# tnestmeyer/reflectance-filtering

Hardware: AMD Instinct MI355X
Metric: megapixels/sec joint-bilateral sigma_c=20 sigma_s=22 @1080p (higher is better)
Workload: dtype f32

## Files before the change

### reflectance_filtering_amd/csrc/rf_jbf.hip

```cpp
#include <algorithm>
#include <atomic>
#include <mutex>
#include <vector>

#include "rf_jbf_common.hpp"
#include "rf_jbf_tables.hpp"
#include "rf_jbf_taploops.hpp"

namespace rf {
namespace {

constexpr int kTileW = 64;
constexpr int kMaxLds = 160 * 1024;
constexpr int kTlw2 = 144;
constexpr int kJbfMaxTiledR4 = 468;
constexpr int kJbfStageOnly = 0x1000, kJbfCompilerLoop = 0x2000, kJbfTile64Only = 0x4000;
constexpr int kJbfLookahead1 = 0x8000;
constexpr int kJbfNoMsad = 0x10000;
constexpr int kJbfVoteOnly = 0x20000;
constexpr int kJbfNoDeadSkip = 0x40000;

int jbf_debug_flags()
{
    return (debug_get(kDbgJbfStageOnly) ? kJbfStageOnly : 0) |
// ... 786 lines not shown
constexpr int kRaggedClasses = 4;
constexpr int kRaggedTh[kRaggedClasses] = {64, 32, 16, 128};
constexpr int kRaggedPitch144[kRaggedClasses] = {144, 208, 336, 136};

struct RaggedPlan {
    bool tiled = false;
    bool slab = false;
    Tile64Shape shape{};
    SlabShape slab_shape{};
    std::vector<JbfTileRec> recs[kRaggedClasses];
};

void plan_ragged(const JbfTables &t, int n, const int *heights, const int *widths, int src_cn,
                 int flags, int tune, RaggedPlan *plan)
{
    const int nz = t.lut_len < 256 * t.joint_cn ? t.lut_len - 1 : t.lut_len;
    if ((flags & RF_JBF_FORCE_GENERIC) || tune != 0)
        return;
    plan->tiled = tile64_choose(t, nz, src_cn, flags, &plan->shape);
    plan->slab = !plan->tiled && slab_choose(t, nz, src_cn, &plan->slab_shape);
    if (!plan->tiled && !plan->slab)
        return;
    const Tile64Shape &s = plan->shape;
    unsigned long long first = 0;
    for (int i = 0; i < n; i++) {
        const int h = heights[i], w = widths[i];
        Tile64Areas a{h, w, 0, 0, 0};
        if (plan->tiled && s.tlw == 144)
            a = tile64_areas(t, nz, s.grep, s.crep, src_cn, flags, h, w);
        const int area[kRaggedClasses][4] = {{0, a.rows_main, 0, a.cols_main},
                                             {a.rows_main, a.s32, 0, a.cols_main},
                                             {a.rows_main + a.s32, a.s16, 0, a.cols_main},
                                             {0, a.sx ? h : 0, a.cols_main, a.sx}};
        for (int c = 0; c < kRaggedClasses; c++) {
            const int th = kRaggedTh[c], tw = 4096 / th;
            for (int y = 0; y < area[c][1]; y += th)
                for (int x = 0; x < area[c][3]; x += tw)
                    plan->recs[c].push_back(
                        JbfTileRec{first, h, w, area[c][0] + y, area[c][2] + x, {0, 0}});
        }
        first += (unsigned long long)h * w;
    }
}

template <int SCN, int GREP, int CREP, int TLW, int TH>
int launch_tile64_ragged(const JbfTables &t, int nz, int crows, const uint8_t *joint,
                         const uint8_t *src, uint8_t *dst, const JbfTileRec *d_recs, size_t ntiles,
                         int jcn, int border, int flags, hipStream_t stream)
{
    if (ntiles == 0)
        return RF_OK;
    if (!launch_fits(ntiles, 1024))
        return fail(RF_E_UNSUPPORTED, "rf_jbf_ragged_u8: too many tiles for one launch");
    auto kern = jbf_tile64_kernel<SCN, GREP, CREP, TLW, TH, true>;
    RF_HIP_CHECK(hipFuncSetAttribute((const void *)kern, hipFuncAttributeMaxDynamicSharedMemorySize,
                                     kT64Lds));
    hipLaunchKernelGGL(kern, dim3((unsigned)ntiles), dim3(1024), kT64Lds, stream, joint, src, dst, 0,
                       0, jcn, t.radius, border, t.d_lut, nz, t.d_hw, t.d_swsym, t.sw_len, d_recs, 0,
                       flags, crows, 0, 0, JbfNoTileFlags{});
    return RF_OK;
}

template <int SCN, int GREP, int CREP, int TLW>
int launch_ragged(const JbfTables &t, int nz, const RaggedPlan &plan, const uint8_t *joint,
                  const uint8_t *src, uint8_t *dst, const JbfTileRec *const *d_recs, int jcn,
                  int border, int flags, hipStream_t stream)
{
    int rc = launch_tile64_ragged<SCN, GREP, CREP, TLW, 64>(t, nz, plan.shape.crows, joint, src, dst,
                                                            d_recs[0], plan.recs[0].size(), jcn,
                                                            border, flags, stream);
    if constexpr (TLW == 144) {
        if (rc == RF_OK)
            rc = launch_tile64_ragged<SCN, GREP, CREP, 208, 32>(t, nz, 32, joint, src, dst, d_recs[1],
                                                                plan.recs[1].size(), jcn, border,
                                                                flags, stream);
        if constexpr (SCN == 1) {
            if (rc == RF_OK)
                rc = launch_tile64_ragged<1, GREP, CREP, 336, 16>(t, nz, 32, joint, src, dst,
                                                                  d_recs[2], plan.recs[2].size(), jcn,
                                                                  border, flags, stream);
            if (rc == RF_OK)
                rc = launch_tile64_ragged<1, GREP, CREP, 136, 128>(t, nz, 32, joint, src, dst,
                                                                   d_recs[3], plan.recs[3].size(),
                                                                   jcn, border, flags, stream);
        }
    }
    return rc;
}

template <int GREP, int TLW, bool kRagged = false>
__global__ __launch_bounds__(1024) void jbf_slab_kernel(
    const uint8_t *__restrict__ joint, const uint8_t *__restrict__ src, uint8_t *__restrict__ dst,
    int h, int w, int jcn, int scn, int radius, int border, const float *__restrict__ lut, int nz,
    const int *__restrict__ hwtab, const float *__restrict__ swsym, int sw_len,
    typename JbfTilesArg<kRagged>::type tiles_x, int tiles_per_img, int flags, int crows_g, int slab_g,
    int crows_c, int slab_c)
{
    constexpr int NT = 1024, Q4 = TLW / 4, QW = 16;
    static_assert(TLW % 32 == 16, "row pitch keeps the rows of a half-wave on disjoint banks");
    extern __shared__ __align__(16) unsigned char smem[];
    int *flag_word = reinterpret_cast<int *>(smem);
    uint32_t *tile4 = reinterpret_cast<uint32_t *>(smem + 16);
    const int tid = threadIdx.x;
    if (tid == 0)
        *flag_word = 3;
    const int tile_id = xcd_contiguous_tile((int)blockIdx.x, (int)gridDim.x);
    int tile_y0, tile_x0;
    size_t img;
    if constexpr (kRagged) {
        const JbfTileRec *rec = tiles_x + tile_id;
        img = (size_t)rec->first;
        h = rec->h;
        w = rec->w;
        tile_y0 = rec->tile_y0;
        tile_x0 = rec->tile_x0;
    } else {
        const int img_idx = tile_id / tiles_per_img;
        const int t_in_img = tile_id - img_idx * tiles_per_img;
        tile_y0 = (t_in_img / tiles_x) * 64;
        tile_x0 = (t_in_img % tiles_x) * 64;
        img = (size_t)img_idx * h * w;
    }
    const int r4 = (radius + 3) & ~3;
    const int tx = tid % QW, ty = tid / QW;
    float *lut_g = reinterpret_cast<float *>(smem + kT64Lds - nz * GREP * 4);
    for (int i = tid; i < nz * GREP; i += NT)
        lut_g[i] = lut[i / GREP];
    const uint32_t lut_lane_addr = lds_addr(lut_g) + (uint32_t)(tid & (GREP - 1)) * 4u;
    const uint32_t tile_lane_addr = lds_addr(tile4) + (uint32_t)tx * 4u;
    int all_grey = scn == 1;
    if (scn == 3) {
        int grey = 1;
        const int rows_all = min(64, h - tile_y0) + 2 * radius;
        for (int item = tid; item < rows_all * Q4; item += NT) {
            const int ry = item / Q4, k = item - ry * Q4;
            const int gy = border_interpolate(tile_y0 - radius + ry, h, border);
            uint32_t jv[4], sv[4];
            load_tile_quad(joint, src, img, gy, tile_x0 - r4 + 4 * k, w, jcn, scn, border, jv, sv);
#pragma unroll
            for (int u = 0; u < 4; u++)
                grey &= (int)(((sv[u] ^ (sv[u] >> 8)) & 0xffffu) == 0u);
        }
        all_grey = __builtin_amdgcn_readfirstlane(block_all2(grey, 1, flag_word) & 1);
    }
    const bool rgb6 = !all_grey && crows_c > 0;
    const int crows = rgb6 ? crows_c : crows_g, slab_rows = rgb6 ? slab_c : slab_g;
    const bool active = tid < QW * crows;
    for (int y0 = tile_y0; y0 < tile_y0 + 64 && y0 < h; y0 += crows) {
        for (int c = 0; c < (all_grey || rgb6 ? 1 : scn); c++) {
            uint32_t jc[kPix];
            float sum1[kPix][1], sum3[kPix][3], wsum[kPix];
            {
                uint32_t jv[4], sv[4];
                load_tile_quad(joint, src, img, min(y0 + ty, h - 1), tile_x0 + 4 * tx, w, jcn, scn, border,
                               jv, sv);
#pragma unroll
                for (int p = 0; p < kPix; p++) {
                    jc[p] = jv[p] & 0x00ffffffu;
                    sum1[p][0] = sum3[p][0] = sum3[p][1] = sum3[p][2] = 0.f;
                    wsum[p] = 0.f;
                }
            }
            const bool msad = !(flags & kJbfNoMsad) && jbf_wave_takes_msad(jc, active);
            for (int i0 = -radius; i0 <= radius; i0 += slab_rows) {
                const int i1 = min(i0 + slab_rows - 1, radius);
                const int tlh = crows + (i1 - i0);
                uint16_t *plane_b = reinterpret_cast<uint16_t *>(tile4 + (size_t)tlh * TLW);
                __syncthreads();
                for (int item = tid; item < tlh * Q4; item += NT) {
                    const int ry = item / Q4, k = item - ry * Q4;
                    const int gy = border_interpolate(y0 + i0 + ry, h, border);
                    uint32_t jv[4], sv[4];
                    load_tile_quad(joint, src, img, gy, tile_x0 - r4 + 4 * k, w, jcn, scn, border, jv, sv);
#pragma unroll
                    for (int u = 0; u < 4; u++) {
                        tile4[ry * TLW + u * Q4 + k] = jv[u] | (((sv[u] >> (8 * c)) & 0xffu) << 24);
                        if (rgb6)
                            plane_b[ry * TLW + u * Q4 + k] = (uint16_t)(sv[u] >> 8);
                    }
                }
                __syncthreads();
                if (active) {
                    if (rgb6 && msad)
                        jbf_tap_loop_rgb6<GREP, TLW, true, true>(lut_lane_addr, swsym, tile_lane_addr,
                                                                 lds_addr(plane_b) + (uint32_t)tx * 2u, jc, ty,
                                                                 radius, r4, sw_len, hwtab, sum3, wsum, i0, i1,
                                                                 -i0);
                    else if (rgb6)
                        jbf_tap_loop_rgb6<GREP, TLW, true>(lut_lane_addr, swsym, tile_lane_addr,
                                                           lds_addr(plane_b) + (uint32_t)tx * 2u, jc, ty,
                                                           radius, r4, sw_len, hwtab, sum3, wsum, i0, i1, -i0);
                    else if (msad)
                        jbf_tap_loop_grey4_la2<GREP, TLW, false, true, true>(lut_lane_addr, swsym,
                                                                             tile_lane_addr, jc, ty, radius, r4,
                                                                             sw_len, hwtab, sum1, wsum, i0, i1,
                                                                             -i0);
                    else
                        jbf_tap_loop_grey4_la2<GREP, TLW, false, true>(lut_lane_addr, swsym, tile_lane_addr,
                                                                       jc, ty, radius, r4, sw_len, hwtab,
                                                                       sum1, wsum, i0, i1, -i0);
                }
            }
            if (active) {
                if (rgb6)
                    store_quad<3, 3>(dst, img, y0 + ty, tile_x0 + 4 * tx, h, w, sum3, wsum, flags);
                else if (scn == 1)
                    store_quad<1, 1>(dst, img, y0 + ty, tile_x0 + 4 * tx, h, w, sum1, wsum, flags);
                else if (all_grey)
                    store_quad<1, 3>(dst, img, y0 + ty, tile_x0 + 4 * tx, h, w, sum1, wsum, flags);
                else
                    store_quad_channel(dst, img, y0 + ty, tile_x0 + 4 * tx, h, w, c, sum1, wsum, flags);
            }
        }
    }
}

void slab_fits(const JbfTables &t, int nz, int grep, int tlw, int texel_bytes, int *crows, int *slab_rows)
{
    *crows = *slab_rows = 0;
    if (2 * t.r4 + 64 + 8 > tlw)
        return;
    const long long rows =
        ((long long)kT64Lds - 16 - (long long)nz * grep * 4) / ((long long)tlw * texel_bytes);
    for (int cr : {64, 32, 16}) {
        const long long sl = rows - cr + 1;
        if (sl >= (cr == 16 ? 8 : 24)) {
            *crows = cr;
            *slab_rows = (int)std::min<long long>(sl, 2 * t.radius + 1);
            return;
        }
    }
}

#define RF_SLAB_PITCHES(X)                                                                    \
    X(68, 208) X(84, 240) X(100, 272) X(116, 304) X(132, 336) X(164, 400) X(212, 496) X(276, 624) \
    X(372, 816) X(kJbfMaxTiledR4, 1008)

bool slab_choose(const JbfTables &t, int nz, int src_cn, SlabShape *out)
{
    if (t.r4 <= 52 || t.r4 > kJbfMaxTiledR4)
        return false;
    SlabShape s{};
#define RF_PITCH(R4_, TLW_) \
    if (!s.tlw && t.r4 <= R4_) \
        s.tlw = TLW_;
    RF_SLAB_PITCHES(RF_PITCH)
#undef RF_PITCH
    for (int g : {16, 8}) {
        int cr, sl;
        slab_fits(t, nz, g, s.tlw, 4, &cr, &sl);
        if (cr > s.crows_g)
            s.crows_g = cr, s.slab_g = sl, s.grep = g;
    }
    if (s.crows_g == 0)
        return false;
    if (src_cn == 3)
        slab_fits(t, nz, s.grep, s.tlw, 6, &s.crows_c, &s.slab_c);
    *out = s;
    return true;
}

template <int GREP, int TLW>
int launch_slab(const JbfTables &t, int nz, int crows, int slab_rows, int crows_c, int slab_c,
                const uint8_t *joint, const uint8_t *src, uint8_t *dst, int n, int h, int w, int jcn,
                int scn, int border, int flags, hipStream_t stream)
{
    const int tiles_x = ceil_div(w, 64), tiles_y = ceil_div(h, 64);
    const long long blocks = (long long)tiles_x * tiles_y * n;
    if (!launch_fits(blocks, 1024))
        return fail(RF_E_UNSUPPORTED, "rf_jbf_u8: batch too large for one launch");
    auto kern = jbf_slab_kernel<GREP, TLW>;
    RF_HIP_CHECK(hipFuncSetAttribute((const void *)kern, hipFuncAttributeMaxDynamicSharedMemorySize,
                                     kT64Lds));
    hipLaunchKernelGGL(kern, dim3((unsigned)blocks), dim3(1024), kT64Lds, stream, joint, src, dst, h,
                       w, jcn, scn, t.radius, border, t.d_lut, nz, t.d_hw, t.d_swsym, t.sw_len,
                       tiles_x, tiles_x * tiles_y, flags, crows, slab_rows, crows_c, slab_c);
    return RF_OK;
}

template <int GREP, int TLW>
int launch_slab_ragged(const JbfTables &t, int nz, const SlabShape &s, const uint8_t *joint,
                       const uint8_t *src, uint8_t *dst, const JbfTileRec *d_recs, size_t ntiles,
                       int jcn, int scn, int border, int flags, hipStream_t stream)
{
    if (ntiles == 0)
        return RF_OK;
    if (!launch_fits(ntiles, 1024))
        return fail(RF_E_UNSUPPORTED, "rf_jbf_ragged_u8: too many tiles for one launch");
    auto kern = jbf_slab_kernel<GREP, TLW, true>;
    RF_HIP_CHECK(hipFuncSetAttribute((const void *)kern, hipFuncAttributeMaxDynamicSharedMemorySize,
                                     kT64Lds));
    hipLaunchKernelGGL(kern, dim3((unsigned)ntiles), dim3(1024), kT64Lds, stream, joint, src, dst, 0,
                       0, jcn, scn, t.radius, border, t.d_lut, nz, t.d_hw, t.d_swsym, t.sw_len,
                       d_recs, 0, flags, s.crows_g, s.slab_g, s.crows_c, s.slab_c);
    return RF_OK;
}

int tile64x2_slab_rows(int nz, int grep, int tlw)
{
    const int rows = (kT64x2Lds - nz * grep * 4) / (tlw * 4);
    return rows >= 64 ? rows - 64 + 1 : 0;
}

template <int GREP, int TLW>
__global__ __launch_bounds__(1024, 8) void jbf_tile64x2_kernel(
    const uint8_t *__restrict__ joint, const uint8_t *__restrict__ src, uint8_t *__restrict__ dst,
    int h, int w, int jcn, int scn, int radius, int border, const float *__restrict__ lut, int nz,
    const int *__restrict__ hwtab, const float *__restrict__ swsym, int sw_len, int tiles_x,
    int tiles_per_img, int flags, int slab_rows, uint8_t *__restrict__ tile_flags)
{
    constexpr int NT = 1024, Q4 = TLW / 4, QW = 16;
    static_assert(TLW % 32 == 16, "row pitch keeps the rows of a half-wave on disjoint banks");
    extern __shared__ __align__(16) unsigned char smem[];
    int *flag_word = reinterpret_cast<int *>(smem);
    uint32_t *tile4 = reinterpret_cast<uint32_t *>(smem);
    const int tid = threadIdx.x;
    if (tid == 0)
        *flag_word = 3;
    __syncthreads();
    const int tile_id = xcd_contiguous_tile((int)blockIdx.x, (int)gridDim.x);
    const int img_idx = tile_id / tiles_per_img;
    const int t_in_img = tile_id - img_idx * tiles_per_img;
    const int tile_y0 = (t_in_img / tiles_x) * 64;
    const int tile_x0 = (t_in_img % tiles_x) * 64;
    const size_t img = (size_t)img_idx * h * w;
    const int r4 = (radius + 3) & ~3;
    const int tx = tid % QW, ty = tid / QW;
    int grey_joint = 1;
    if (flags & kJbfVoteOnly) {
        int grey = 1;
        const int rows_all = 64 + 2 * radius;
        for (int item = tid; item < rows_all * Q4; item += NT) {
            const int ry = item / Q4, k = item - ry * Q4;
            const int gy = border_interpolate(tile_y0 - radius + ry, h, border);
            uint32_t jv[4], sv[4];
            load_tile_quad(joint, src, img, gy, tile_x0 - r4 + 4 * k, w, jcn, scn, border, jv, sv);
#pragma unroll
            for (int u = 0; u < 4; u++) {
                if (scn == 3)
                    grey &= (int)(((sv[u] ^ (sv[u] >> 8)) & 0xffffu) == 0u);
                if (jcn == 3)
                    grey_joint &= (int)(((jv[u] ^ (jv[u] >> 8)) & 0xffffu) == 0u);
            }
        }
        const int bits = block_all2(grey, grey_joint, flag_word);
        if (tid == 0)
            tile_flags[tile_id] = (uint8_t)(((bits & 1) ? 0 : 1) | (bits & 2));
        return;
    }
    if (tile_flags) {
        const int byte = __builtin_amdgcn_readfirstlane((int)tile_flags[tile_id]);
        if (byte & 1)
            return;
        grey_joint = (byte >> 1) & 1;
    }
    float *lut_g = reinterpret_cast<float *>(smem + kT64x2Lds - nz * GREP * 4);
    for (int i = tid; i < nz * GREP; i += NT)
        lut_g[i] = lut[i / GREP];
    const uint32_t lut_lane_addr = lds_addr(lut_g) + (uint32_t)(tid & (GREP - 1)) * 4u;
    const uint32_t tile_lane_addr = lds_addr(tile4) + (uint32_t)tx * 4u;
    const bool j1 = grey_joint != 0;
    const uint32_t j1_scale = (uint32_t)(jcn == 1 ? 1 : 3) * (GREP * 4u);
    uint32_t jc[kPix];
    float sum1[kPix][1], wsum[kPix];
    {
        uint32_t jv[4], sv[4];
        load_tile_quad(joint, src, img, border_interpolate(tile_y0 + ty, h, border), tile_x0 + 4 * tx, w, jcn,
                       scn, border, jv, sv);
#pragma unroll
        for (int p = 0; p < kPix; p++) {
            jc[p] = j1 ? (jv[p] & 0xffu) * j1_scale : jv[p] & 0x00ffffffu;
            sum1[p][0] = 0.f;
            wsum[p] = 0.f;
        }
    }
    const bool msad = !j1 && !(flags & kJbfNoMsad) && jbf_wave_takes_msad(jc);
    const bool live_wave =
        __builtin_amdgcn_readfirstlane(tile_y0 + (ty & ~3)) < h || (flags & kJbfNoDeadSkip) != 0;
    for (int i0 = -radius; i0 <= radius; i0 += slab_rows) {
        const int i1 = min(i0 + slab_rows - 1, radius);
        const int tlh = 64 + (i1 - i0);
        __syncthreads();
        for (int item = tid; item < tlh * Q4; item += NT) {
            const int ry = item / Q4, k = item - ry * Q4;
            const int gy = border_interpolate(tile_y0 + i0 + ry, h, border);
            uint32_t jv[4], sv[4];
            load_tile_quad(joint, src, img, gy, tile_x0 - r4 + 4 * k, w, jcn, scn, border, jv, sv);
#pragma unroll
            for (int u = 0; u < 4; u++) {
                const uint32_t jfield = j1 ? (jv[u] & 0xffu) * j1_scale : jv[u];
                tile4[ry * TLW + u * Q4 + k] = jfield | (sv[u] << 24);
            }
        }
        __syncthreads();
        if (!live_wave)
            continue;
        if (j1)
            jbf_tap_loop_grey4_la2<GREP, TLW, true, true>(lut_lane_addr, swsym, tile_lane_addr, jc, ty,
                                                          radius, r4, sw_len, hwtab, sum1, wsum, i0, i1, -i0);
        else if (msad)
            jbf_tap_loop_grey4_la2<GREP, TLW, false, true, true>(lut_lane_addr, swsym, tile_lane_addr, jc,
                                                                 ty, radius, r4, sw_len, hwtab, sum1, wsum,
                                                                 i0, i1, -i0);
        else
            jbf_tap_loop_grey4_la2<GREP, TLW, false, true>(lut_lane_addr, swsym, tile_lane_addr, jc, ty,
                                                           radius, r4, sw_len, hwtab, sum1, wsum, i0, i1,
                                                           -i0);
    }
    if (scn == 1)
        store_quad<1, 1>(dst, img, tile_y0 + ty, tile_x0 + 4 * tx, h, w, sum1, wsum, flags);
    else
        store_quad<1, 3>(dst, img, tile_y0 + ty, tile_x0 + 4 * tx, h, w, sum1, wsum, flags);
}

struct TileFlagBuf {
    int dev;
    hipStream_t stream;
    uint8_t *p;
    size_t bytes;
};
std::mutex g_tf_mu;
std::vector<TileFlagBuf> g_tf;
std::vector<uint8_t *> g_tf_retired;
constexpr size_t kTileFlagStreams = 16;
std::atomic<int> g_two_wg_calls{0};

size_t tile_flag_bytes(size_t tiles)
{
    size_t b = 4096;
    while (b < tiles)
        b <<= 1;
    return b;
}

int get_tile_flags(int dev, hipStream_t stream, size_t tiles, uint8_t **out)
{
    *out = nullptr;
    std::lock_guard<std::mutex> lock(g_tf_mu);
    size_t at = g_tf.size();
    for (size_t i = 0; i < g_tf.size(); i++)
        if (g_tf[i].dev == dev && g_tf[i].stream == stream)
            at = i;
    if (at < g_tf.size() && g_tf[at].bytes >= tiles) {
        *out = g_tf[at].p;
        return RF_OK;
    }
    hipStreamCaptureStatus st = hipStreamCaptureStatusNone;
    if (hipStreamIsCapturing(stream, &st) != hipSuccess || st != hipStreamCaptureStatusNone) {
        (void)hipGetLastError();
        return RF_OK;
    }
    if (at == g_tf.size() && g_tf.size() >= kTileFlagStreams)
        return RF_OK;
    uint8_t *p = nullptr;
    {
        CaptureRelax relax;
        RF_HIP_CHECK(hipMalloc(&p, tile_flag_bytes(tiles)));
    }
    if (at < g_tf.size()) {
        g_tf_retired.push_back(g_tf[at].p);
        g_tf.erase(g_tf.begin() + at);
    }
    g_tf.push_back(TileFlagBuf{dev, stream, p, tile_flag_bytes(tiles)});
    *out = p;
    return RF_OK;
}

bool two_wg_choose(const JbfTables &t, int nz, int src_cn, int flags, int *slab_rows)
{
    *slab_rows = 0;
    if (debug_get(kDbgJbfNoTwoWg) || debug_get(kDbgJbfTune) ||
        (flags & (RF_JBF_FORCE_GENERIC | kJbfStageOnly | kJbfCompilerLoop | kJbfLookahead1)))
        return false;
    Tile64Shape shape;
    if (t.r4 > 36 || !tile64_choose(t, nz, src_cn, flags, &shape) || shape.tlw != 144 || shape.grep != 32)
        return false;
    *slab_rows = tile64x2_slab_rows(nz, 32, 144);
    return *slab_rows >= 8;
}

int launch_tile64x2(const JbfTables &t, int nz, int slab_rows, const uint8_t *joint, const uint8_t *src,
                    uint8_t *dst, int n, int h, int w, int jcn, int scn, int border, int flags,
                    hipStream_t stream, int rows, int cols, uint8_t *tile_flags)
{
    const int tiles_x = ceil_div(cols, 64), tiles_y = ceil_div(rows, 64);
    const long long blocks = (long long)tiles_x * tiles_y * n;
    auto kern = jbf_tile64x2_kernel<32, 144>;
    RF_HIP_CHECK(hipFuncSetAttribute((const void *)kern, hipFuncAttributeMaxDynamicSharedMemorySize,
                                     kT64x2Lds));
    hipLaunchKernelGGL(kern, dim3((unsigned)blocks), dim3(1024), kT64x2Lds, stream, joint, src, dst, h, w,
                       jcn, scn, t.radius, border, t.d_lut, nz, t.d_hw, t.d_swsym, t.sw_len, tiles_x,
                       tiles_x * tiles_y, flags, slab_rows, tile_flags);
    return RF_OK;
}

template <int CREP>
int launch_tile64_flagged(const JbfTables &t, int nz, int crows, const uint8_t *joint, const uint8_t *src,
                          uint8_t *dst, int n, int h, int w, int jcn, int border, int flags,
                          hipStream_t stream, int rows, int cols, const uint8_t *tile_flags)
{
    const int tiles_x = ceil_div(cols, 64), tiles_y = ceil_div(rows, 64);
    const long long blocks = (long long)tiles_x * tiles_y * n;
    auto kern = jbf_tile64_kernel<3, 32, CREP, 144, 64, false, true>;
    RF_HIP_CHECK(hipFuncSetAttribute((const void *)kern, hipFuncAttributeMaxDynamicSharedMemorySize,
                                     kT64Lds));
    hipLaunchKernelGGL(kern, dim3((unsigned)blocks), dim3(1024), kT64Lds, stream, joint, src, dst, h, w,
                       jcn, t.radius, border, t.d_lut, nz, t.d_hw, t.d_swsym, t.sw_len, tiles_x,
                       tiles_x * tiles_y, flags, crows, 0, 0, tile_flags);
    return RF_OK;
}

int launch_two_wg(const JbfTables &t, int nz, const Tile64Shape &shape, int slab_rows,
                  const uint8_t *joint, const uint8_t *src, uint8_t *dst, int n, int h, int w, int jcn,
                  int scn, int border, int flags, hipStream_t stream, bool *done)
{
    *done = false;
    const Tile64Areas a = tile64_areas(t, nz, shape.grep, shape.crep, scn, flags, h, w);
    if (a.rows_main <= 0 || a.cols_main <= 0)
        return RF_OK;
    const long long blocks = (long long)ceil_div(a.cols_main, 64) * ceil_div(a.rows_main, 64) * n;
    if (!launch_fits(blocks, 1024))
        return fail(RF_E_UNSUPPORTED, "rf_jbf_u8: batch too large for one launch");
    uint8_t *tile_flags = nullptr;
    int rc = RF_OK;
    if (scn == 3 || jcn == 3) {
        if (int bad = get_tile_flags(t.device, stream, (size_t)blocks, &tile_flags))
            return bad;
        if (!tile_flags)
            return RF_OK;
        const int tiles_x = ceil_div(a.cols_main, 64), tiles_y = ceil_div(a.rows_main, 64);
        if (debug_get(kDbgJbfVoteScan) || !jbf_grey_map_serves(h, w, t.radius, border, tiles_x, tiles_y))
            rc = launch_tile64x2(t, nz, slab_rows, joint, src, dst, n, h, w, jcn, scn, border,
                                 flags | kJbfVoteOnly, stream, a.rows_main, a.cols_main, tile_flags);
        else
            rc = jbf_launch_grey_map(joint, src, n, h, w, jcn, scn, t.radius, border, stream, tiles_x, tiles_y,
                                     tile_flags);
    }
    if (rc == RF_OK && scn == 3)
        rc = shape.crep == 32 ? launch_tile64_flagged<32>(t, nz, shape.crows, joint, src, dst, n, h, w, jcn,
                                                          border, flags, stream, a.rows_main, a.cols_main,
                                                          tile_flags)
                              : launch_tile64_flagged<16>(t, nz, shape.crows, joint, src, dst, n, h, w, jcn,
                                                          border, flags, stream, a.rows_main, a.cols_main,
                                                          tile_flags);
    if (rc == RF_OK)
        rc = launch_tile64x2(t, nz, slab_rows, joint, src, dst, n, h, w, jcn, scn, border, flags, stream,
                             a.rows_main, a.cols_main, tile_flags);
    if (rc == RF_OK && (a.s32 || a.s16 || a.sx)) {
        if (scn == 3)
            rc = shape.crep == 32 ? launch_tile64_rows<3, 32, 32>(t, nz, shape.crows, joint, src, dst, n, h, w,
                                                                  jcn, border, flags, stream, true)
                                  : launch_tile64_rows<3, 32, 16>(t, nz, shape.crows, joint, src, dst, n, h, w,
                                                                  jcn, border, flags, stream, true);
        else
            rc = shape.crep == 32 ? launch_tile64_rows<1, 32, 32>(t, nz, shape.crows, joint, src, dst, n, h, w,
                                                                  jcn, border, flags, stream, true)
                                  : launch_tile64_rows<1, 32, 16>(t, nz, shape.crows, joint, src, dst, n, h, w,
                                                                  jcn, border, flags, stream, true);
    }
    *done = rc == RF_OK;
    if (*done)
        g_two_wg_calls.fetch_add(1, std::memory_order_relaxed);
    return rc;
}

}

void jbf_scratch_release()
{
    std::lock_guard<std::mutex> lock(g_tf_mu);
    for (const TileFlagBuf &b : g_tf)
        (void)hipFree(b.p);
    for (uint8_t *p : g_tf_retired)
        (void)hipFree(p);
    g_tf.clear();
    g_tf_retired.clear();
}

}

extern "C" int rf_debug_jbf_two_wg_calls(void)
{
    return rf::g_two_wg_calls.load(std::memory_order_relaxed) & 0x7fffffff;
}

extern "C" int rf_debug_jbf_tile_flags(void *stream_, unsigned char *out, int cap)
{
    using namespace rf;
    hipStream_t stream = (hipStream_t)stream_;
    if (cap < 0 || (!out && cap))
        return fail(RF_E_BADARG, "rf_debug_jbf_tile_flags: NULL out or a negative cap");
    if (stream_is_capturing(stream))
        return fail(RF_E_UNSUPPORTED, "rf_debug_jbf_tile_flags: synchronises its stream and cannot be "
                                      "captured into a graph");
    int dev = 0;
    RF_HIP_CHECK(hipGetDevice(&dev));
    const uint8_t *p = nullptr;
    size_t bytes = 0;
    {
        std::lock_guard<std::mutex> lock(g_tf_mu);
        for (const TileFlagBuf &b : g_tf)
            if (b.dev == dev && b.stream == stream)
                p = b.p, bytes = b.bytes;
    }
    if (bytes > (size_t)cap)
        bytes = (size_t)cap;
    if (bytes) {
        RF_HIP_CHECK(hipMemcpyAsync(out, p, bytes, hipMemcpyDeviceToHost, stream));
        RF_HIP_CHECK(hipStreamSynchronize(stream));
    }
    return (int)bytes;
}

extern "C" int rf_jbf_release_scratch(void)
{
    rf::jbf_scratch_release();
    return RF_OK;
}

extern "C" int rf_jbf_u8(const uint8_t *joint, const uint8_t *src, uint8_t *dst, int n, int h,
                         int w, int joint_cn, int src_cn, int d, double sigma_color,
                         double sigma_space, int border, int flags, void *stream_)
{
    using namespace rf;
    if (n == 0)
        return RF_OK;
    if (!joint || !src || !dst)
        return fail(RF_E_BADARG, "rf_jbf_u8: NULL image pointer");
    if (n < 0 || h <= 0 || w <= 0)
        return fail(RF_E_BADARG, "rf_jbf_u8: bad size n=%d h=%d w=%d", n, h, w);
    if (int bad = jbf_check_format("rf_jbf_u8", joint_cn, src_cn, border))
        return bad;
    {
        const size_t px = (size_t)n * h * w;
        if (ranges_overlap(dst, px * src_cn, joint, px * joint_cn) ||
            ranges_overlap(dst, px * src_cn, src, px * src_cn))
            return fail(RF_E_BADARG, "rf_jbf_u8: dst must not overlap an input");
    }
    if (flags & ~kJbfPublicFlags)
        return fail(RF_E_BADARG, "rf_jbf_u8: unknown flag bits 0x%x", flags);
    flags |= jbf_debug_flags();
    sigma_color = jbf_sigma(sigma_color);
    sigma_space = jbf_sigma(sigma_space);
    const int radius = jbf_radius(d, sigma_space);
    if (radius > kJbfMaxRadius)
        return fail(RF_E_UNSUPPORTED, "rf_jbf_u8: radius %d too large", radius);
    hipStream_t stream = (hipStream_t)stream_;
    const int jcn_kernel = jbf_kernel_cn(joint_cn, flags);
    joint_cn = jbf_table_cn(joint_cn, flags);
    JbfTables t;
    TablesHold hold{t};
    int rc = get_tables(radius, joint_cn, sigma_color, sigma_space, stream, &t);
    if (rc != RF_OK)
        return rc;

    const int tune = debug_get(kDbgJbfTune) & 0xf;
    static const Tiled2Config kCfg[] = {{48, 16, false}, {32, 8, true},  {32, 32, false},
                                        {32, 16, false}, {64, 16, false}, {48, 8, false}};
    constexpr int kNumCfg = (int)(sizeof(kCfg) / sizeof(kCfg[0]));
    bool done = false;
    if (!(flags & RF_JBF_FORCE_GENERIC) && t.r4 <= kJbfMaxTiledR4 && (tune == 0 || tune == 7)) {
        bool oob_ok = false, oob_half = false;
        rc = lds_oob_reads_zero(t.device, &oob_ok, &oob_half);
        if (rc != RF_OK)
            return rc;
        const int nz = t.lut_len < 256 * joint_cn ? t.lut_len - 1 : t.lut_len;
        if (oob_ok) {
            Tile64Shape shape;
            if (tile64_choose(t, nz, src_cn, flags, &shape)) {
                int slab2 = 0;
                if (oob_half && two_wg_choose(t, nz, src_cn, flags, &slab2)) {
                    rc = launch_two_wg(t, nz, shape, slab2, joint, src, dst, n, h, w, jcn_kernel, src_cn,
                                       border, flags, stream, &done);
                    if (rc != RF_OK)
                        return rc;
                }
#define RF_T64(G_, C_, W_)                                                                        \
    if (!done && shape.grep == G_ && shape.crep == C_ && shape.tlw == W_) {                       \
        if (W_ == 144)                                                                            \
            rc = src_cn == 3 ? launch_tile64_rows<3, G_, C_>(t, nz, shape.crows, joint, src, dst, \
                                                             n, h, w, jcn_kernel, border, flags,  \
                                                             stream)                              \
                             : launch_tile64_rows<1, G_, C_>(t, nz, shape.crows, joint, src, dst, \
                                                             n, h, w, jcn_kernel, border, flags,  \
                                                             stream);                             \
        else                                                                                      \
            rc = src_cn == 3 ? launch_tile64<3, G_, C_, W_>(t, nz, shape.crows, joint, src, dst,  \
                                                            n, h, w, jcn_kernel, border, flags,   \
                                                            stream)                               \
                             : launch_tile64<1, G_, C_, W_>(t, nz, shape.crows, joint, src, dst,  \
                                                            n, h, w, jcn_kernel, border, flags,   \
                                                            stream);                              \
    }
                RF_T64_SHAPES(RF_T64)
#undef RF_T64
                if (rc != RF_OK)
// ... 316 lines not shown
```

Baseline: 2748.

## Stage tile rows with raw wide loads, byte-perm packing, and row lookahead

Replaces the generic per-item staging loop with a per-thread column routine. For interior columns it issues raw 4/12-byte loads for several rows ahead, then packs joint and source bytes into tile words with alignbyte/perm; edge columns fall back to the per-pixel path. It also writes the replicated LUT to LDS as float4 stores instead of scalar stores. The aim is to cut global load instruction count and latency stalls in the slab staging phase, at the cost of more complex packing logic whose byte-select masks must be correct for every channel combination.

```diff
diff --git a/reflectance_filtering_amd/csrc/rf_jbf.hip b/reflectance_filtering_amd/csrc/rf_jbf.hip
--- a/reflectance_filtering_amd/csrc/rf_jbf.hip
+++ b/reflectance_filtering_amd/csrc/rf_jbf.hip
@@ -1112,6 +1112,115 @@
     return rows >= 64 ? rows - 64 + 1 : 0;
 }
 
+__device__ inline void load_raw4(const uint8_t *p, int cn, uint32_t (&d)[3])
+{
+    if (cn == 3)
+        __builtin_memcpy(&d[0], p, 12);
+    else
+        __builtin_memcpy(&d[0], p, 4);
+}
+
+__device__ inline void pack_tile_words(const uint32_t (&jr)[3], const uint32_t (&sr)[3], int jcn, int scn, bool j1,
+                                       uint32_t j1_scale, uint32_t (&wd)[4])
+{
+    const uint32_t s0 = sr[0], s1 = sr[0], s2 = scn == 3 ? sr[1] : sr[0], s3 = scn == 3 ? sr[2] : sr[0];
+    if (jcn == 3 && !j1) {
+        const uint32_t t1 = __builtin_amdgcn_alignbyte(jr[1], jr[0], 3);
+        const uint32_t t2 = __builtin_amdgcn_alignbyte(jr[2], jr[1], 2);
+        if (scn == 3) {
+            wd[0] = __builtin_amdgcn_perm(s0, jr[0], 0x04020100u);
+            wd[1] = __builtin_amdgcn_perm(s1, t1, 0x07020100u);
+            wd[2] = __builtin_amdgcn_perm(s2, t2, 0x06020100u);
+            wd[3] = __builtin_amdgcn_perm(s3, jr[2], 0x05030201u);
+        } else {
+            wd[0] = __builtin_amdgcn_perm(s0, jr[0], 0x04020100u);
+            wd[1] = __builtin_amdgcn_perm(s1, t1, 0x05020100u);
+            wd[2] = __builtin_amdgcn_perm(s2, t2, 0x06020100u);
+            wd[3] = __builtin_amdgcn_perm(s3, jr[2], 0x07030201u);
+        }
+        return;
+    }
+    uint32_t jb[4];
+    if (jcn == 3) {
+        jb[0] = jr[0] & 0xffu;
+        jb[1] = jr[0] >> 24;
+        jb[2] = (jr[1] >> 16) & 0xffu;
+        jb[3] = (jr[2] >> 8) & 0xffu;
+    } else {
+        jb[0] = jr[0] & 0xffu;
+        jb[1] = (jr[0] >> 8) & 0xffu;
+        jb[2] = (jr[0] >> 16) & 0xffu;
+        jb[3] = jr[0] >> 24;
+    }
+    const uint32_t mul = j1 ? j1_scale : (jcn < 0 ? 0x010101u : 1u);
+    if (scn == 3) {
+        wd[0] = __builtin_amdgcn_perm(s0, jb[0] * mul, 0x04020100u);
+        wd[1] = __builtin_amdgcn_perm(s1, jb[1] * mul, 0x07020100u);
+        wd[2] = __builtin_amdgcn_perm(s2, jb[2] * mul, 0x06020100u);
+        wd[3] = __builtin_amdgcn_perm(s3, jb[3] * mul, 0x05020100u);
+    } else {
+        wd[0] = __builtin_amdgcn_perm(s0, jb[0] * mul, 0x04020100u);
+        wd[1] = __builtin_amdgcn_perm(s1, jb[1] * mul, 0x05020100u);
+        wd[2] = __builtin_amdgcn_perm(s2, jb[2] * mul, 0x06020100u);
+        wd[3] = __builtin_amdgcn_perm(s3, jb[3] * mul, 0x07020100u);
+    }
+}
+
+template <int TLW>
+__device__ inline void stage_tile_rows(uint32_t *tile4, const uint8_t *joint, const uint8_t *src, size_t img,
+                                       int y_first, int tlh, int x_left, int h, int w, int jcn, int scn,
+                                       int border, bool j1, uint32_t j1_scale, int tid)
+{
+    constexpr int Q4 = TLW / 4, RP = 1024 / Q4, kAhead = 3;
+    int j1_form = j1;
+    asm volatile("" : "+v"(tid), "+s"(jcn), "+s"(scn), "+s"(j1_form));
+    j1 = j1_form != 0;
+    const int r0 = tid / Q4, k = tid - r0 * Q4;
+    if (r0 >= RP)
+        return;
+    const int x_first = x_left + 4 * k;
+    uint32_t *out = tile4 + r0 * TLW + k;
+    if (x_first >= 0 && x_first + 3 < w) {
+        const uint32_t jb = jcn == 3 ? 3u : 1u, sb = scn == 3 ? 3u : 1u;
+        const uint8_t *jp = joint + (img + (size_t)x_first) * jb, *sp = src + (img + (size_t)x_first) * sb;
+        const uint32_t jrow = (uint32_t)w * jb, srow = (uint32_t)w * sb;
+        for (int ry = r0; ry < tlh; ry += kAhead * RP, out += kAhead * RP * TLW) {
+            uint32_t jr[kAhead][3], sr[kAhead][3];
+#pragma unroll
+            for (int a = 0; a < kAhead; a++) {
+                if (ry + a * RP >= tlh)
+                    continue;
+                const uint32_t gy = (uint32_t)max(border_interpolate(y_first + ry + a * RP, h, border), 0);
+                load_raw4(jp + (size_t)gy * jrow, jcn, jr[a]);
+                load_raw4(sp + (size_t)gy * srow, scn, sr[a]);
+            }
+#pragma unroll
+            for (int a = 0; a < kAhead; a++)
+                if (ry + a * RP < tlh) {
+                    uint32_t wd[4];
+                    pack_tile_words(jr[a], sr[a], jcn, scn, j1, j1_scale, wd);
+                    if (border == RF_BORDER_CONSTANT && (unsigned)(y_first + ry + a * RP) >= (unsigned)h)
+                        wd[0] = wd[1] = wd[2] = wd[3] = 0u;
+#pragma unroll
+                    for (int u = 0; u < 4; u++)
+                        out[a * RP * TLW + u * Q4] = wd[u];
+                }
+        }
+        return;
+    }
+    for (int ry = r0; ry < tlh; ry += RP, out += RP * TLW) {
+        const int gy = border_interpolate(y_first + ry, h, border);
+        const size_t row = img + (size_t)(gy < 0 ? 0 : gy) * w;
+#pragma unroll 1
+        for (int u = 0; u < 4; u++) {
+            const int gx = gy < 0 ? -1 : border_interpolate(x_first + u, w, border);
+            const uint32_t jv = gx < 0 ? 0u : load_packed(joint, row + gx, jcn);
+            const uint32_t sv = gx < 0 ? 0u : load_packed(src, row + gx, scn);
+            out[u * Q4] = (j1 ? (jv & 0xffu) * j1_scale : jv) | (sv << 24);
+        }
+    }
+}
+
 template <int GREP, int TLW>
 __global__ __launch_bounds__(1024, 8) void jbf_tile64x2_kernel(
     const uint8_t *__restrict__ joint, const uint8_t *__restrict__ src, uint8_t *__restrict__ dst,
@@ -1165,8 +1274,11 @@
         grey_joint = (byte >> 1) & 1;
     }
     float *lut_g = reinterpret_cast<float *>(smem + kT64x2Lds - nz * GREP * 4);
-    for (int i = tid; i < nz * GREP; i += NT)
-        lut_g[i] = lut[i / GREP];
+    static_assert(GREP % 4 == 0 && kT64x2Lds % 16 == 0, "the LUT's replicas go out as 16-byte stores");
+    for (int i = tid; i < nz * (GREP / 4); i += NT) {
+        const float v = lut[i / (GREP / 4)];
+        reinterpret_cast<float4 *>(lut_g)[i] = make_float4(v, v, v, v);
+    }
     const uint32_t lut_lane_addr = lds_addr(lut_g) + (uint32_t)(tid & (GREP - 1)) * 4u;
     const uint32_t tile_lane_addr = lds_addr(tile4) + (uint32_t)tx * 4u;
     const bool j1 = grey_joint != 0;
@@ -1191,17 +1303,8 @@
         const int i1 = min(i0 + slab_rows - 1, radius);
         const int tlh = 64 + (i1 - i0);
         __syncthreads();
-        for (int item = tid; item < tlh * Q4; item += NT) {
-            const int ry = item / Q4, k = item - ry * Q4;
-            const int gy = border_interpolate(tile_y0 + i0 + ry, h, border);
-            uint32_t jv[4], sv[4];
-            load_tile_quad(joint, src, img, gy, tile_x0 - r4 + 4 * k, w, jcn, scn, border, jv, sv);
-#pragma unroll
-            for (int u = 0; u < 4; u++) {
-                const uint32_t jfield = j1 ? (jv[u] & 0xffu) * j1_scale : jv[u];
-                tile4[ry * TLW + u * Q4 + k] = jfield | (sv[u] << 24);
-            }
-        }
+        stage_tile_rows<TLW>(tile4, joint, src, img, tile_y0 + i0, tlh, tile_x0 - r4, h, w, jcn, scn, border, j1,
+                             j1_scale, tid);
         __syncthreads();
         if (!live_wave)
             continue;
```

New measurement: 2757 (median of 6 runs). Within noise of the previous version (+0.3%).
